# jcorsetti/oryon

Hardware: AMD Instinct MI355X
Metric: image-pairs/sec end-to-end (feat+match+reg) @224², C=256; ADD(-S) parity (higher is better)
Workload: dtype f32

## Files before the change

oryon_amd/csrc/match_corrs.hip:

```cpp
#include <hip/hip_fp16.h>
#include "common.h"
#include "match_common.h"
#include "match_exact.h"

namespace oryon {
constexpr uint8_t LZ_INVALID = 0, LZ_VALID = 1, LZ_UNCERTAIN = 2, LZ_AMB_VALID = 3, LZ_RESOLVED = 4, LZ_AMB_UNCERTAIN = 5;
constexpr uint8_t DC_COMPLETE = 0, DC_SETTLED = 1, DC_OPEN = 2;

struct DcOpenRows {
    const uint8_t *cls = nullptr;
    int S = 0;
    const float *m1 = nullptr;
    const int32_t *i1 = nullptr;
    const float *m2 = nullptr;
    float *r_m1 = nullptr;
    int32_t *r_i1 = nullptr;
    float *r_m2 = nullptr;
};

__device__ __forceinline__ bool decide_lite_row(
    int cap_a, int p, int a, int S, const float *ws_m1, const int32_t *ws_i1,
    const float *ws_m2, const DcOpenRows &open, const float *__restrict__ a_scale8, const float *__restrict__ eps_q8, float cut0, float sqrt_c,
    float c_true, int force_eager, int fmt, int x3, float *__restrict__ m_final, int32_t *__restrict__ sid_final, float *__restrict__ margin_out,
    uint8_t *__restrict__ state, uint8_t *__restrict__ valid, float *__restrict__ min_dist, int32_t *__restrict__ argmin,
// ... 596 lines not shown
    return carve.off;
}

size_t carve_lazy(void *base, LazyWs &w, int B, int C, int cap_a, int cap_q, int S, int corr_rows)
{
    Carver carve(base, carve_screen8_raw(base, w, B, C, cap_a, cap_q, S));
    const size_t rows = (size_t)B * cap_a, pairs = (size_t)B;
    carve(w.margin, rows);
    carve(w.sid_final, rows);
    carve(w.unc_idx, rows);
    carve(w.state, rows);
    carve(w.sel_rows, pairs * corr_rows);
    carve(w.scratch, rows);
    carve(w.n_a_eager, pairs);
    carve(w.n_a_lazy, pairs);
    carve(w.ambu_idx, rows);
    carve(w.ambv_idx, pairs * corr_rows);
    const size_t cap_s = sampled_cap(corr_rows, cap_a);
    const size_t e1 = oryon_match_workspace_bytes(B, cap_a), e2 = oryon_match_workspace_bytes(B, (int)cap_s);
    w.exact_ws_bytes = e1 > e2 ? e1 : e2;
    carve(w.exact_ws, w.exact_ws_bytes > 16 ? w.exact_ws_bytes : 16);
    carve(w.x3_ah, pairs * cap_s * C);
    carve(w.x3_al, pairs * cap_s * C);
    carve(w.x3_a_ovf, pairs * cap_s * C);
    carve(w.x3_md_o, pairs * cap_s);
    carve(w.x3_am_o, pairs * cap_s);
    carve(w.x3_va_o, pairs * cap_s);
    const bool cascade = C == 256 && corr_rows <= MX6_SAMPLED_PANEL;
    const size_t triples = cascade ? pairs * mx6_sampled_splits(B) * MX6_SAMPLED_PANEL : 4;
    carve(w.cs_panel, cascade ? pairs * MX6_SAMPLED_PANEL * C : 16);
    if (!cascade) w.cs_panel = nullptr;
    carve(w.cs_max, triples);
    carve(w.cs_m2, triples);
    carve(w.cs_i1, triples);
    carve(w.n_ambv0, pairs);
    carve(w.cs_gate, pairs * mx6_panels_per_pair(cap_a));
    w.dc_ok = false;
    w.dc_stats = nullptr;
    if (dc_shape(C, cap_a, corr_rows)) {
        LazyWs sized;
        if (carve_dc(nullptr, sized, B, C, cap_a) <= (size_t)B * cap_q * C * sizeof(__half)) {
            carve_dc(w.q16, w, B, C, cap_a);
            w.dc_ok = true;
        }
    }
    w.lazy_zero_off = carve.off;
    carve(w.pair_eager, pairs);
    carve(w.n_unc, pairs);
    carve(w.n_ambu, pairs);
    carve(w.n_ambv, pairs);
    carve(w.need_f32_lazy, pairs);
    carve(w.n_amb_room, pairs);
    w.n_amb_part = w.panel_flag;
    carve(w.mark, rows);
    w.lazy_zero_bytes = carve.off - w.lazy_zero_off;
    w.x3_zero_bytes = match_x3_zero_bytes(B, (int)cap_s, 8);
    carve(w.x3_scratch, match_x3_scratch_bytes(B, (int)cap_s, 8, cap_q));
    return carve.off;
}
}

extern "C" size_t oryon_match_corrs_i8_workspace_bytes(int B, int C, int cap_a, int cap_q, int corr_rows)
{
    if (B <= 0 || C <= 0 || cap_a <= 0 || cap_a % MT16 || cap_q <= 0 || corr_rows <= 0) return 0;
    LazyWs w;
    return carve_lazy(nullptr, w, B, C, cap_a, cap_q, pick_split16(B, cap_a / MT16), corr_rows);
}

int32_t *oryon::match_dc_stats(void *workspace, int B, int C, int cap_a, int cap_q, int corr_rows)
{
    LazyWs w;
    carve_lazy(workspace, w, B, C, cap_a, cap_q, pick_split16(B, cap_a / MT16), corr_rows);
    return w.dc_ok ? w.dc_stats : nullptr;
}

namespace {
constexpr const char *IMPL = "match_corrs_lazy_impl";

SampledAmbList sampled_amb_list(const LazyWs &w)
{
    SampledAmbList L;
    L.state = w.state;
    L.want = LZ_AMB_VALID;
    L.mark = w.mark;
    L.n_list = w.n_ambv;
    L.list = w.ambv_idx;
    return L;
}

int select_step(const MatchCorrsArgs &m, const LazyWs &w, hipStream_t st, const SampledAmbList &amb = SampledAmbList())
{
    const int rc = select_corrs_launch(m.roi_a, m.roi_q, m.roi_stride_a, m.roi_stride_q, m.n_a, m.n_q, m.argmin, m.valid, m.cap_a, m.B, m.W,
                                       m.max_corrs, m.corr_rows, m.seed, m.pair_key, w.scratch, m.corrs, m.n_valid, m.n_sel, m.status,
                                       w.sel_rows, w.pair_eager, st, amb);
    if (rc) set_error("oryon_match_corrs_i8: select launch failed");
    return rc;
}

int eager_route(const MatchCorrsArgs &m, const LazyWs &w, int S)
{
    decide8_step(m, S, w.n_a_eager, w);
    rescore_raw_step(m, w.n_a_eager, 2, w);
    int rc = check_launch(IMPL);
    if (rc) return rc;
    if ((rc = raw_fallbacks(m, w.n_a_eager, w, IMPL, "oryon_match_corrs_i8"))) return rc;
    return select_step(m, w, as_stream(m.stream));
}

void compact_anchors(const MatchCorrsArgs &m, const AnchorRaw &araw, const LazyWs &w, hipStream_t st, int cap_c, const int32_t *count,
                     const int32_t *idx, int idx_stride)
{
    const dim3 grid((cap_c + 63) / 64, m.B);
    if (m.a_hat)
        hipLaunchKernelGGL(match_compact_f32_kernel, grid, dim3(256), 0, st, m.a_hat, m.C, m.cap_a, cap_c, count, idx, idx_stride, w.a_hat_c);
    else
        hipLaunchKernelGGL(m.layout == ORYON_LAYOUT_NHWC ? match_compact_raw_kernel<true> : match_compact_raw_kernel<false>, grid, dim3(256), 0,
                           st, araw, m.C_true, m.HW, m.round_f16, m.C, m.cap_a, cap_c, count, idx, idx_stride, w.a_hat_c);
}

int lazy_route(const MatchCorrsArgs &m, const LazyWs &w, hipStream_t st, int use_x3, bool cascade, bool dc)
{
    const int B = m.B, C = m.C, cap_a = m.cap_a, cap_q = m.cap_q, corr_rows = m.corr_rows;
    const bool nhwc = m.layout == ORYON_LAYOUT_NHWC;
    const AnchorRaw araw = {m.feat_a, m.roi_a, m.a_norm, m.roi_stride_a};
    int rc = gather_q8_launch(m.feat_q, B, m.C_true, m.HW, m.layout, m.roi_q, m.roi_stride_q, m.n_q, w.need_f32_lazy, cap_q, C, w.q8_scratch,
                              w.scale_scratch, w.eps_scratch, nullptr, w.q_hat, 1, m.round_f16, st);
    if (rc) { set_error("oryon_match_corrs_i8: lazy fp32 gather launch failed"); return rc; }
    compact_anchors(m, araw, w, st, cap_a, w.n_ambu, w.ambu_idx, cap_a);
    if ((rc = check_launch(IMPL))) return rc;
    rc = oryon_match_f32(w.a_hat_c, w.q_hat, B, C, cap_a, cap_q, w.n_ambu, m.n_q, m.threshold, w.md_c, w.am_c, w.va_c, w.exact_ws,
                         w.exact_ws_bytes, st);
    if (rc) return rc;
    hipLaunchKernelGGL(match_scatter_exact_kernel, dim3(cap_a / 256, B), dim3(256), 0, st, cap_a, cap_a, w.n_ambu, w.ambu_idx, cap_a, w.md_c,
                       w.am_c, w.va_c, m.min_dist, m.argmin, m.valid, w.state);
    if ((rc = check_launch(IMPL))) return rc;
    const size_t lds_res = (size_t)4 * 2 * C * sizeof(float);
    auto resolve_uncertain = m.fmt == 1 ? (nhwc ? match_resolve_uncertain_kernel<true, 1> : match_resolve_uncertain_kernel<false, 1>)
                                        : (nhwc ? match_resolve_uncertain_kernel<true, 0> : match_resolve_uncertain_kernel<false, 0>);
    hipLaunchKernelGGL(resolve_uncertain, dim3(64, B), dim3(256), lds_res, st, m.a_hat, araw, m.a_i8, m.q_i8, m.q_scale, m.a_scale, m.feat_q,
                       m.C_true, m.HW, m.roi_q, m.roi_stride_q, m.q_norm, C, cap_a, cap_q, m.n_q, m.threshold, w.m_final, w.sid_final, w.margin,
                       w.n_unc, w.unc_idx, w.pair_eager, w.state, m.valid, m.min_dist, m.argmin, m.round_f16);
    if ((rc = check_launch(IMPL))) return rc;
    const SampledAmbList amb = sampled_amb_list(w);
    if ((rc = select_step(m, w, st, amb))) return rc;
    const int cap_s = sampled_cap(corr_rows, cap_a);
    if (cascade) {
        const int csS = mx6_sampled_splits(B);
        launch_screen_mx6_list512(st, reinterpret_cast<const uint8_t *>(m.a_i8), reinterpret_cast<const uint8_t *>(m.q_i8), B, cap_a, MX6_SAMPLED_PANEL,
                                  cap_q, w.n_ambv, w.ambv_idx, corr_rows, 0, m.n_q, csS, w.cs_max, w.cs_i1, w.cs_m2, m.C_true);
        hipLaunchKernelGGL(match_decide_sampled_kernel, dim3(B), dim3(DS_THREADS), 0, st, cap_a, MX6_SAMPLED_PANEL, csS,
                           w.n_ambv, w.ambv_idx, corr_rows, w.cs_max, w.cs_i1, w.cs_m2, m.a_scale, m.q_eps_max, w.m_final, w.sid_final,
                           w.margin, w.state, w.mark, w.n_ambv0, dc ? m.min_dist : nullptr, w.pair_eager, m.n_sel, w.sel_rows, amb);
        if ((rc = check_launch(IMPL))) return rc;
    }
    compact_anchors(m, araw, w, st, cap_s, w.n_ambv, w.ambv_idx, corr_rows);
    if ((rc = check_launch(IMPL))) return rc;
    if (use_x3) {
        __half *qh = reinterpret_cast<__half *>(w.q_hat), *ql = qh + (size_t)B * cap_q * C;
        int32_t *n_ovf = nullptr, *ovf_idx = nullptr;
        rc = match_x3_resolve(w.a_hat_c, w.n_ambv, cap_s, m.feat_q, m.C_true, m.HW, m.layout, m.roi_q, m.roi_stride_q, m.q_norm, m.n_q, B, cap_q,
                              m.threshold, m.round_f16, qh, ql, w.x3_ah, w.x3_al, w.x3_scratch, w.md_c, w.am_c, w.va_c, &n_ovf, &ovf_idx,
                              w.ambv_idx, corr_rows, w.sid_final, cap_a, static_cast<const __half *>(m.q_hi_lo), m.q_lo_sq_max, st);
        if (rc) { set_error("oryon_match_corrs: fp16x3 second-level launch failed"); return rc; }
        rc = gather_q8_launch(m.feat_q, B, m.C_true, m.HW, m.layout, m.roi_q, m.roi_stride_q, m.n_q, n_ovf, cap_q, C, w.q8_scratch,
                              w.scale_scratch, w.eps_scratch, nullptr, w.q_hat, 1, m.round_f16, st);
        if (rc) { set_error("oryon_match_corrs: overflow fp32 gather launch failed"); return rc; }
        hipLaunchKernelGGL(match_compact_f32_kernel, dim3((cap_s + 63) / 64, B), dim3(256), 0, st, w.a_hat_c, C, cap_s, cap_s, n_ovf, ovf_idx,
                           cap_s, w.x3_a_ovf);
        if ((rc = check_launch(IMPL))) return rc;
        rc = oryon_match_f32(w.x3_a_ovf, w.q_hat, B, C, cap_s, cap_q, n_ovf, m.n_q, m.threshold, w.x3_md_o, w.x3_am_o, w.x3_va_o, w.exact_ws,
                             w.exact_ws_bytes, st);
        if (rc) return rc;
        match_x3_scatter_ovf(B, cap_s, n_ovf, ovf_idx, w.x3_md_o, w.x3_am_o, w.x3_va_o, w.md_c, w.am_c, w.va_c, st);
    } else {
        rc = oryon_match_f32(w.a_hat_c, w.q_hat, B, C, cap_s, cap_q, w.n_ambv, m.n_q, m.threshold, w.md_c, w.am_c, w.va_c, w.exact_ws,
                             w.exact_ws_bytes, st);
        if (rc) return rc;
    }
    hipLaunchKernelGGL(match_scatter_exact_kernel, dim3((cap_s + 255) / 256, B), dim3(256), 0, st, cap_a, cap_s, w.n_ambv, w.ambv_idx,
                       corr_rows, w.md_c, w.am_c, w.va_c, m.min_dist, m.argmin, m.valid, w.state);
    if ((rc = check_launch(IMPL))) return rc;
    auto resolve_selected = m.fmt == 1 ? (nhwc ? match_resolve_selected_kernel<true, 1> : match_resolve_selected_kernel<false, 1>)
                                       : (nhwc ? match_resolve_selected_kernel<true, 0> : match_resolve_selected_kernel<false, 0>);
    hipLaunchKernelGGL(resolve_selected, dim3((m.max_corrs + 3) / 4, B), dim3(256), lds_res, st, m.a_hat, araw, m.a_i8, m.q_i8, m.q_scale,
                       m.a_scale, m.feat_q, m.C_true, m.HW, m.roi_q, m.roi_stride_q, m.q_norm, C, cap_a, cap_q, m.n_q, m.W, w.m_final,
                       w.sid_final, w.margin, w.state, w.pair_eager, m.n_sel, w.sel_rows, corr_rows, m.min_dist, m.argmin, m.corrs,
                       m.round_f16);
    if ((rc = check_launch(IMPL))) return rc;
    if (m.n_undecided && cascade) {
        hipLaunchKernelGGL(match_cascade_counts_kernel, dim3((B + 255) / 256), dim3(256), 0, st, B, w.n_amb_part, cap_a / 256, w.n_ambv, w.n_ambv0,
                           m.n_undecided);
        if ((rc = check_launch(IMPL))) return rc;
    } else if (m.n_undecided) {
        hipLaunchKernelGGL(match_sum_counts_kernel, dim3((B + 255) / 256), dim3(256), 0, st, B, w.n_amb, w.n_amb_part, cap_a / 256,
                           m.n_undecided);
        if ((rc = check_launch(IMPL))) return rc;
    }
    return ORYON_OK;
}
}

int oryon::match_corrs_lazy_impl(const MatchCorrsArgs &m)
{
    ORYON_CHECK_ARG((m.a_hat || (m.feat_a && m.a_norm && !m.force_eager)) && m.a_i8 && m.a_scale && m.feat_q && m.roi_a && m.roi_q && m.q_norm && m.q_i8 && m.q_eps_max && m.n_a && m.n_q);
    ORYON_CHECK_ARG((m.fmt == 0 || m.fmt == 1) && (m.fmt == 1 || m.q_scale) && !(m.fmt == 1 && m.force_eager));
    ORYON_CHECK_ARG(!m.q_hi_lo || (m.q_lo_sq_max && m.C == 256));
    ORYON_CHECK_ARG(m.min_dist && m.argmin && m.valid && m.corrs && m.n_valid && m.n_sel && m.status);
    ORYON_CHECK_ARG(m.B >= 0 && (m.C == 256 || m.C == 512) && m.C_true > 0 && m.C_true <= m.C && m.HW > 0 && m.W > 0 && m.max_corrs > 0 && m.corr_rows >= m.max_corrs);
    ORYON_CHECK_ARG(m.layout == ORYON_LAYOUT_NCHW || m.layout == ORYON_LAYOUT_NHWC);
    ORYON_CHECK_ARG(m.cap_a > 0 && m.cap_a % MT16 == 0 && m.cap_q > 0 && m.cap_q % 256 == 0 && m.threshold > 0.0f && m.threshold <= 0.5f);
    if (m.B == 0) return ORYON_OK;
    const int B = m.B, C = m.C, cap_a = m.cap_a, cap_q = m.cap_q;
    const int T = cap_a / MT16;
    const int S = pick_split16(B, T);
    LazyWs w;
    const size_t need = carve_lazy(m.workspace, w, B, C, cap_a, cap_q, S, m.corr_rows);
    if (!m.workspace || m.workspace_bytes < need) {
        set_error("oryon_match_corrs_i8: workspace too small (%zu < %zu)", m.workspace_bytes, need);
        return ORYON_ERR_WORKSPACE;
    }
    hipStream_t st = as_stream(m.stream);
    const float cut0 = 1.0f - 2.0f * m.threshold;
    static const bool x3_env = dev_env_int("ORYON_AMB_X3", 1) != 0;
    const int use_x3 = (x3_env && C == 256 && !m.force_eager) ? 1 : 0;
    ORYON_CHECK_HIP(hipMemsetAsync(static_cast<char *>(m.workspace) + w.zero_off, 0, w.zero_bytes + (w.dc_ok && m.fmt == 1 ? w.dc_zero_bytes : 0), st));
    if (m.force_eager) ORYON_CHECK_HIP(hipMemsetAsync(w.need_f32, 0, (size_t)B * sizeof(int32_t), st));
    ORYON_CHECK_HIP(hipMemsetAsync(static_cast<char *>(m.workspace) + w.lazy_zero_off, 0, w.lazy_zero_bytes + (use_x3 ? w.x3_zero_bytes : 0), st));
    static const bool cascade_env = dev_env_int("ORYON_CASCADE", 1) != 0;
    const bool cascade = cascade_env && m.fmt == 1 && use_x3 && m.q_hi_lo != nullptr && w.cs_panel != nullptr;
    const bool dc = m.cascade != 0 && m.fmt == 1 && use_x3 && m.q_hi_lo == nullptr && w.cs_panel != nullptr && w.dc_ok;
    int S_dec = S;
    const float *dec_m1 = w.ws_max, *dec_m2 = w.ws_m2;
    const int32_t *dec_i1 = w.ws_i1;
    DcOpenRows dc_open;
    if (m.fmt == 1) {
        const uint8_t *a6 = reinterpret_cast<const uint8_t *>(m.a_i8), *q6 = reinterpret_cast<const uint8_t *>(m.q_i8);
        const int groups = ((B * S + 7) / 8) * 8 * T;
        profile_begin(st, screen_mx6_name(C));
        if (cascade) {
            const int T8 = mx6_panels_per_pair(cap_a);
            launch_screen_mx6(C, groups, T, st, a6, q6, B, cap_a, cap_q, m.n_a, m.n_q, S, w.ws_max, w.ws_i1, w.ws_m2, m.C_true, 1, nullptr, 2);
            hipLaunchKernelGGL(match_panel_settle_kernel, dim3(T8, B), dim3(256), 0, st, cap_a, T8, S, m.n_a, w.ws_max, w.ws_m2, m.a_scale,
                               m.q_eps_max, cut0, w.cs_gate);
            launch_screen_mx6(C, groups, T, st, a6, q6, B, cap_a, cap_q, m.n_a, m.n_q, S, w.ws_max, w.ws_i1, w.ws_m2, m.C_true, 1, w.cs_gate, 0);
        } else if (dc) {
            const int T8 = mx6_panels_per_pair(cap_a), stride = dc_probe_stride(cap_a), csS = mx6_sampled_splits(B);
            const int Sb = dc_band_splits(B, cap_a), So = dc_open_splits(B);
            static const int slack = dev_env_int("ORYON_DC_SLACK", DC_SLACK);
            static const int open_panel = dev_env_int("ORYON_DC_OPEN_PANEL", 0) == 1024 ? 1024 : MX6_SAMPLED_PANEL;
            static const int sub_stats = dev_env_int("ORYON_DC_SUB_STATS", 0);
            launch_screen_mx6_list512(st, a6, q6, B, cap_a, MX6_SAMPLED_PANEL, cap_q, m.n_a, nullptr, 0, stride, m.n_q, csS, w.cs_max, w.cs_i1,
                                      w.cs_m2, m.C_true);
            hipLaunchKernelGGL(match_dc_probe_band_kernel, dim3(T8, B), dim3(256), 0, st, cap_a, T8, stride, csS, m.n_a, m.n_q, w.cs_max, w.cs_i1,
                               w.cs_m2, m.a_scale, m.q_eps_max, cut0, w.dc_m1, w.dc_i1, w.dc_m2, w.dc_band, w.dc_stats, slack, sub_stats);
            launch_screen_mx6_band512(st, a6, q6, B, cap_a, cap_q, m.n_a, m.n_q, Sb, w.dc_ws_m1, w.dc_ws_i1, w.dc_ws_m2, m.C_true, w.dc_band, 2 * T8);
            hipLaunchKernelGGL(match_dc_settle_rows_kernel, dim3(B), dim3(DC_SETTLE_THREADS), 0, st, cap_a, T8, stride, Sb, m.n_a, m.n_q, w.dc_ws_m1, w.dc_ws_i1,
                               w.dc_ws_m2, m.a_scale, m.q_eps_max, cut0, w.dc_band, w.dc_m1, w.dc_i1, w.dc_m2, w.dc_cls, w.dc_n_open, w.dc_open_idx,
                               w.dc_stats);
            if (open_panel == 1024) {
                hipLaunchKernelGGL(match_compact_rows_kernel, dim3(cap_a / 16, B), dim3(256), 0, st, a6, C, cap_a, cap_a, w.dc_n_open, w.dc_open_idx,
                                   cap_a, w.dc_rows, open_panel);
                launch_screen_mx6(C, ((B * So + 7) / 8) * 8 * T, T, st, w.dc_rows, q6, B, cap_a, cap_q, w.dc_n_open, m.n_q, So, w.dc_ws_m1, w.dc_ws_i1,
                                  w.dc_ws_m2, m.C_true);
            } else
                launch_screen_mx6_list512(st, a6, q6, B, cap_a, cap_a, cap_q, w.dc_n_open, w.dc_open_idx, cap_a, 0, m.n_q, So, w.dc_ws_m1, w.dc_ws_i1,
                                          w.dc_ws_m2, m.C_true);
            S_dec = 1;
            dec_m1 = w.dc_m1; dec_i1 = w.dc_i1; dec_m2 = w.dc_m2;
            dc_open.cls = w.dc_cls;
            dc_open.S = So;
            dc_open.m1 = w.dc_ws_m1; dc_open.i1 = w.dc_ws_i1; dc_open.m2 = w.dc_ws_m2;
            dc_open.r_m1 = w.dc_m1; dc_open.r_i1 = w.dc_i1; dc_open.r_m2 = w.dc_m2;
        } else {
            launch_screen_mx6(C, groups, T, st, a6, q6, B, cap_a, cap_q, m.n_a, m.n_q, S, w.ws_max, w.ws_i1, w.ws_m2, m.C_true);
        }
        profile_end(st);
    } else {
        screen8_step(m, S, m.n_a, w);
    }
    ORYON_CHECK_LAUNCH();
    hipLaunchKernelGGL(match_decide_lite_kernel, dim3(cap_a / 256, B), dim3(256), 0, st, cap_a, m.n_a, S_dec, dec_m1, dec_i1, dec_m2, dc_open, m.a_scale,
                       m.q_eps_max, cut0, sqrtf((float)m.C_true), (float)m.C_true, m.force_eager, m.fmt, use_x3, w.m_final, w.sid_final, w.margin,
                       w.state, m.valid, m.min_dist, m.argmin, w.pair_eager, w.n_unc, w.unc_idx, w.n_ambu, w.ambu_idx, w.need_f32_lazy,
                       w.n_amb_part);
    if (m.force_eager)
        hipLaunchKernelGGL(match_mask_counts_kernel, dim3((B + 255) / 256), dim3(256), 0, st, B, m.n_a, w.pair_eager, w.n_a_eager, w.n_a_lazy);
    ORYON_CHECK_LAUNCH();
    if (!m.force_eager) return lazy_route(m, w, st, use_x3, cascade || dc, dc);
    const int rc = eager_route(m, w, S);
    if (rc) return rc;
    if (m.n_undecided) ORYON_CHECK_HIP(hipMemcpyAsync(m.n_undecided, w.n_amb, (size_t)B * sizeof(int32_t), hipMemcpyDeviceToDevice, st));
    return ORYON_OK;
}

namespace {
MatchCorrsArgs shared_args(const float *feat_q, int C_true, int HW, int layout, const int32_t *roi_a, int roi_stride_a, const int32_t *roi_q,
                           int roi_stride_q, const float *q_norm, int B, int C, int cap_a, int cap_q, const int32_t *n_a, const int32_t *n_q,
                           float threshold, int W, int max_corrs, int corr_rows, uint64_t seed, const int64_t *pair_key, float *min_dist,
                           int32_t *argmin, uint8_t *valid, int32_t *corrs, int32_t *n_valid, int32_t *n_sel, int32_t *status,
                           int32_t *n_undecided, int round_f16, void *workspace, size_t workspace_bytes, void *stream)
{
    MatchCorrsArgs m;
    m.feat_q = feat_q;
    m.C_true = C_true;
    m.HW = HW;
    m.layout = layout;
// ... 169 lines not shown
```

oryon_amd/csrc/screen_mx6.hip:

```cpp
#include <hip/hip_runtime.h>
#include <stdio.h>
#include <stdlib.h>
#include <type_traits>
#include "common.h"
#include "match_common.h"
#include "screen_tile.h"

namespace oryon {

typedef int i32x8 __attribute__((ext_vector_type(8)));
typedef float f32x16s __attribute__((ext_vector_type(16)));

template <int CP, int WAVES = 8, int VAR = 0>
__global__ __launch_bounds__(64 * WAVES, CP == 512 ? 1 : 2) void match_mx6_screen_kernel(
    const uint8_t *__restrict__ a6, const uint8_t *__restrict__ q6, int B, int cap_a, int cap_q, const int32_t *__restrict__ n_a,
    const int32_t *__restrict__ n_q, int T, int S, float *__restrict__ ws_max, int32_t *__restrict__ ws_i1, float *__restrict__ ws_m2)
{
    constexpr int RB = CP;
    constexpr int TILE_BYTES = screen8_tile_bytes(CP);
    constexpr int NQB = 4, NAB = 2;
    constexpr int NKS = CP / 64;
    constexpr int NI = TILE_BYTES / (1024 * WAVES);
    char *smem;
    if constexpr (2 * TILE_BYTES > 65536) {
        extern __shared__ __attribute__((aligned(256))) char smem_dyn6[];
        smem = smem_dyn6;
    } else {
        __shared__ __attribute__((aligned(256))) char smem_st6[2 * TILE_BYTES];
        smem = smem_st6;
    }
    ScreenUnit u;
    if (!screen_unit_decode(u, 64 * WAVES, B, T, S, n_a, n_q)) return;
    const int p = u.p, split = u.split, a0 = u.a0;
    int qt_begin, qt_end;
    screen_split_tiles(u, S, qt_begin, qt_end);
    const int t = threadIdx.x, lane = t & 63, wave = t >> 6, l31 = lane & 31, hi = lane >> 5;
    const char *qp = reinterpret_cast<const char *>(q6) + (size_t)p * cap_q * RB;

    i32x8 breg[NAB][NKS];
#pragma unroll
    for (int ab = 0; ab < NAB; ++ab) {
        const int arow_i = a0 + wave * 64 + ab * 32 + l31;
        const char *arow = reinterpret_cast<const char *>(a6) + ((size_t)p * cap_a + (arow_i < cap_a ? arow_i : cap_a - 1)) * RB + 32 * hi;
#pragma unroll
        for (int s = 0; s < NKS; ++s) {
            const i32x4 lo = *reinterpret_cast<const i32x4 *>(arow + 64 * s), up = *reinterpret_cast<const i32x4 *>(arow + 64 * s + 16);
            breg[ab][s] = __builtin_shufflevector(lo, up, 0, 1, 2, 3, 4, 5, 6, 7);
        }
    }
    unsigned dma_off[NI];
    screen_dma_offsets<RB>(dma_off, wave * NI, lane);
    const int wave_u = __builtin_amdgcn_readfirstlane(wave);
    auto issue_one = [&](int qt, int buf, int j) {
        const char *qb = qp + (size_t)qt * TILE_BYTES;
        char *dst = smem + buf * TILE_BYTES + (wave_u * NI + j) * 1024;
        __builtin_amdgcn_global_load_lds((const __attribute__((address_space(1))) void *)(qb + dma_off[j]),
                                         (__attribute__((address_space(3))) void *)dst, 16, 0, 0);
    };
    unsigned koff[4][2];
#pragma unroll
    for (int c = 0; c < 4; ++c)
#pragma unroll
        for (int e = 0; e < 2; ++e) koff[c][e] = (unsigned)(l31 * RB) + ((((unsigned)(4 * c + 2 * hi + e)) ^ (unsigned)(l31 & 15)) << 4);
    auto rd = [&](int s, int qb, unsigned tile) -> i32x8 {
        const unsigned base = tile + (unsigned)(qb * 32 * RB + (s >> 2) * 256);
        const i32x4 lo = *reinterpret_cast<const i32x4 *>(smem + koff[s & 3][0] + base);
        const i32x4 up = *reinterpret_cast<const i32x4 *>(smem + koff[s & 3][1] + base);
        return __builtin_shufflevector(lo, up, 0, 1, 2, 3, 4, 5, 6, 7);
    };

    float runmax[NAB], run2[NAB];
    int runidx[NAB];
#pragma unroll
    for (int ab = 0; ab < NAB; ++ab) { runmax[ab] = -INFINITY; run2[ab] = -INFINITY; runidx[ab] = 0; }
    auto reduce_block = [&](const f32x16s &c, int sid, int ab) {
        if constexpr (VAR == 1) { runmax[ab] = fmaxf(runmax[ab], c[0] + c[15]); runidx[ab] = sid; return; }
        const float m0 = fmaxf(fmaxf(c[0], c[1]), c[2]), m1 = fmaxf(fmaxf(c[3], c[4]), c[5]), m2 = fmaxf(fmaxf(c[6], c[7]), c[8]);
        const float m3 = fmaxf(fmaxf(c[9], c[10]), c[11]), m4 = fmaxf(fmaxf(c[12], c[13]), c[14]);
        const float x = fmaxf(fmaxf(fmaxf(m0, m1), m2), fmaxf(fmaxf(m3, m4), c[15]));
        const bool improved = x > runmax[ab];
        run2[ab] = __builtin_amdgcn_fmed3f(runmax[ab], run2[ab], x);
        runmax[ab] = fmaxf(runmax[ab], x);
        runidx[ab] = improved ? sid : runidx[ab];
    };
    const f32x16s zero16 = {0, 0, 0, 0, 0, 0, 0, 0, 0, 0, 0, 0, 0, 0, 0, 0};

    if (qt_end > qt_begin) {
#pragma unroll
        for (int j = 0; j < NI; ++j) issue_one(qt_begin, 0, j);
    }
    asm volatile("s_waitcnt vmcnt(0)" ::: "memory");
    __syncthreads();

    i32x8 areg[NKS];
#pragma unroll
    for (int s = 0; s < NKS; ++s) areg[s] = rd(s, 0, 0u);
    f32x16s prev[NAB];
#pragma unroll
    for (int ab = 0; ab < NAB; ++ab)
#pragma unroll
        for (int r = 0; r < 16; ++r) prev[ab][r] = -3.0e38f;
    int prev_sid = 0;
    auto do_tile = [&](int qt, auto BUFC) {
        constexpr int BUF = decltype(BUFC)::value;
        constexpr unsigned tile = BUF * TILE_BYTES;
        const int qt_next = qt + 1 < qt_end ? qt + 1 : qt;
#pragma unroll
        for (int qb = 0; qb < NQB; ++qb) {
            f32x16s acc[NAB];
            if (qb == 0) {
#pragma unroll
                for (int j = 0; j < NI; ++j) issue_one(qt_next, BUF ^ 1, j);
            }
#pragma unroll
            for (int s = 0; s < NKS; ++s) {
#pragma unroll
                for (int ab = 0; ab < NAB; ++ab)
                    acc[ab] = __builtin_amdgcn_mfma_scale_f32_32x32x64_f8f6f4(areg[s], breg[ab][s], s == 0 ? zero16 : acc[ab], 2, 2, 0,
                                                                               areg[s][6], 0, breg[ab][s][6]);
                if (qb + 1 < NQB) areg[s] = rd(s, qb + 1, tile);
            }
#pragma unroll
            for (int ab = 0; ab < NAB; ++ab) reduce_block(prev[ab], prev_sid, ab);
#pragma unroll
            for (int i = 0; i < NKS; ++i) {
                __builtin_amdgcn_sched_group_barrier(0x008, 1, 0);
                __builtin_amdgcn_sched_group_barrier(0x002, 24 / (2 * NKS), 0);
                __builtin_amdgcn_sched_group_barrier(0x008, 1, 0);
                __builtin_amdgcn_sched_group_barrier(0x002, 24 / (2 * NKS), 0);
                if (qb + 1 < NQB) __builtin_amdgcn_sched_group_barrier(0x100, 2, 0);
            }
#pragma unroll
            for (int ab = 0; ab < NAB; ++ab) prev[ab] = acc[ab];
            prev_sid = (qt * NQB + qb) * 2 + hi;
        }
        asm volatile("s_waitcnt vmcnt(0)" ::: "memory");
        __syncthreads();
#pragma unroll
        for (int s = 0; s < NKS; ++s) areg[s] = rd(s, 0, (BUF ^ 1) * TILE_BYTES);
    };
    for (int qt = qt_begin; qt < qt_end; qt += 2) {
        do_tile(qt, std::integral_constant<int, 0>{});
        if (qt + 1 < qt_end) do_tile(qt + 1, std::integral_constant<int, 1>{});
    }
#pragma unroll
    for (int ab = 0; ab < NAB; ++ab) reduce_block(prev[ab], prev_sid, ab);
    screen_merge_store<NAB>(runmax, run2, runidx, a0 + wave * 64 + l31, hi, (size_t)p * S + split, cap_a, ws_max, ws_i1, ws_m2);
}


template <int S0, int N, class F>
__device__ __forceinline__ void mx6_static_for(F &&f)
{
    if constexpr (S0 < N) {
        f(std::integral_constant<int, S0>{});
        mx6_static_for<S0 + 1, N>(f);
    }
}

struct Mx6RowList {
    const int32_t *idx;
    int idx_stride, stride, cap_src;
    int n;
};
struct Mx6RowsInPlace {};

template <int CP, int WAVES, int KL, bool IDX = false>
__device__ __forceinline__ void mx6_screen_w4_tiles(char *smem, const uint8_t *__restrict__ a6, const uint8_t *__restrict__ q6, int p, int split,
                                                    int a0, int cap_a, int cap_q, int S, int qt_begin, int qt_end, float *__restrict__ ws_max,
                                                    int32_t *__restrict__ ws_i1, float *__restrict__ ws_m2,
                                                    const std::conditional_t<IDX, Mx6RowList, Mx6RowsInPlace> &rows = {})
{
    static_assert(CP == 256 || (CP == 512 && WAVES == 4), "geometries: C_pad 256 with 4 / 8 waves, C_pad 512 with 4 waves");
    constexpr int RB = CP, NAB = 4;
    constexpr int TILE_BYTES = screen8_tile_bytes(CP);
    constexpr int NQB = 4;
    constexpr int NKS = CP / 64;
    constexpr int NI = TILE_BYTES / (1024 * WAVES);
    constexpr int LPR = RB / 256;
    const int t = threadIdx.x, lane = t & 63, wave = t >> 6, l31 = lane & 31, hi = lane >> 5;
    const char *qp = reinterpret_cast<const char *>(q6) + (size_t)p * cap_q * RB;

    i32x8 breg[NAB][NKS];
    int bsc[NAB][NKS / 4];
#pragma unroll
    for (int ab = 0; ab < NAB; ++ab) {
        const int arow_i = a0 + wave * (32 * NAB) + ab * 32 + l31;
        const char *arow;
        bool live = true;
        if constexpr (IDX) {
            live = arow_i < rows.n;
            const int src = !live ? 0 : rows.idx ? rows.idx[(size_t)p * rows.idx_stride + arow_i] : arow_i * rows.stride;
            arow = reinterpret_cast<const char *>(a6) + ((size_t)p * rows.cap_src + src) * RB + 32 * hi;
        } else
            arow = reinterpret_cast<const char *>(a6) + ((size_t)p * cap_a + (arow_i < cap_a ? arow_i : cap_a - 1)) * RB + 32 * hi;
        unsigned sc[NKS / 4];
#pragma unroll
        for (int w = 0; w < NKS / 4; ++w) sc[w] = 0;
#pragma unroll
        for (int s = 0; s < KL; ++s) {
            i32x4 lo = *reinterpret_cast<const i32x4 *>(arow + 64 * s), up = *reinterpret_cast<const i32x4 *>(arow + 64 * s + 16);
            if constexpr (IDX) {
                const i32x4 z = {0, 0, 0, 0};
                lo = live ? lo : z;
                up = live ? up : z;
            }
            breg[ab][s] = __builtin_shufflevector(lo, up, 0, 1, 2, 3, 4, 5, -1, -1);
            sc[s >> 2] |= ((unsigned)up[2] & 0xffu) << (8 * (s & 3));
        }
#pragma unroll
        for (int w = 0; w < NKS / 4; ++w) bsc[ab][w] = (int)sc[w];
    }
    constexpr int DJ = 4 * LPR;
    static_assert(NI % DJ == 0 || NI == DJ, "DMA instructions per wave and tile");
    unsigned dma_off[DJ];
    screen_dma_offsets<RB>(dma_off, wave * NI, lane);
    const int wave_u = __builtin_amdgcn_readfirstlane(wave);
    auto issue_one = [&](int qt, int buf, int j) {
        const char *qb = qp + (size_t)qt * TILE_BYTES + (j / DJ) * (16 * RB);
        char *dst = smem + buf * TILE_BYTES + (wave_u * NI + j) * 1024;
        __builtin_amdgcn_global_load_lds((const __attribute__((address_space(1))) void *)(qb + dma_off[j % DJ]),
                                         (__attribute__((address_space(3))) void *)dst, 16, 0, 0);
    };
    unsigned koff[4][2];
#pragma unroll
    for (int c = 0; c < 4; ++c)
#pragma unroll
        for (int e = 0; e < 2; ++e) koff[c][e] = (unsigned)(l31 * RB) + ((((unsigned)(4 * c + 2 * hi + e)) ^ (unsigned)(l31 & 15)) << 4);
    auto rd = [&](int s, int qb, unsigned tile) -> i32x8 {
        const unsigned base = tile + (unsigned)(qb * 32 * RB + (s >> 2) * 256);
        const i32x4 lo = *reinterpret_cast<const i32x4 *>(smem + koff[s & 3][0] + base);
        const i32x4 up = *reinterpret_cast<const i32x4 *>(smem + koff[s & 3][1] + base);
        return __builtin_shufflevector(lo, up, 0, 1, 2, 3, 4, 5, 6, -1);
    };

    float runmax[NAB], run2[NAB];
    int runidx[NAB];
#pragma unroll
    for (int ab = 0; ab < NAB; ++ab) { runmax[ab] = -INFINITY; run2[ab] = -INFINITY; runidx[ab] = 0; }
    auto reduce_block = [&](const f32x16s &c, int sid, int ab) {
        const float m0 = fmaxf(fmaxf(c[0], c[1]), c[2]), m1 = fmaxf(fmaxf(c[3], c[4]), c[5]), m2 = fmaxf(fmaxf(c[6], c[7]), c[8]);
        const float m3 = fmaxf(fmaxf(c[9], c[10]), c[11]), m4 = fmaxf(fmaxf(c[12], c[13]), c[14]);
        const float x = fmaxf(fmaxf(fmaxf(m0, m1), m2), fmaxf(fmaxf(m3, m4), c[15]));
        const bool improved = x > runmax[ab];
        run2[ab] = __builtin_amdgcn_fmed3f(runmax[ab], run2[ab], x);
        runmax[ab] = __builtin_amdgcn_fmed3f(runmax[ab], x, INFINITY);
        runidx[ab] = improved ? sid : runidx[ab];
    };
    const f32x16s zero16 = {0, 0, 0, 0, 0, 0, 0, 0, 0, 0, 0, 0, 0, 0, 0, 0};

    if (qt_end > qt_begin) {
#pragma unroll
        for (int j = 0; j < NI; ++j) issue_one(qt_begin, 0, j);
    }
    asm volatile("s_waitcnt vmcnt(0)" ::: "memory");
    __syncthreads();

    i32x8 areg[NKS];
#pragma unroll
    for (int s = 0; s < KL; ++s) areg[s] = rd(s, 0, 0u);
    f32x16s acc[NAB];
#pragma unroll
    for (int ab = 0; ab < NAB; ++ab)
#pragma unroll
        for (int r = 0; r < 16; ++r) acc[ab][r] = -3.0e38f;
    int sid23 = 0;

    auto mfma = [&](f32x16s &d, int ab, auto SC) {
        constexpr int s_ = decltype(SC)::value;
        d = __builtin_amdgcn_mfma_scale_f32_32x32x64_f8f6f4(areg[s_], breg[ab][s_], s_ == 0 ? zero16 : d, 2, 2, 0, areg[s_][6], s_ & 3,
                                                            bsc[ab][s_ >> 2]);
    };
    int buf = 0;
    for (int qt = qt_begin; qt < qt_end; ++qt) {
        const unsigned tile = buf * TILE_BYTES;
        const int qt_next = qt + 1 < qt_end ? qt + 1 : qt;
#pragma unroll
        for (int qb = 0; qb < NQB; ++qb) {
            const int sid = (qt * NQB + qb) * 2 + hi;
            if (qb == 0) {
#pragma unroll
                for (int j = 0; j < NI; ++j) issue_one(qt_next, buf ^ 1, j);
            }
            reduce_block(acc[2], sid23, 2);
            reduce_block(acc[3], sid23, 3);
            mx6_static_for<0, KL>([&](auto SC) { mfma(acc[0], 0, SC); mfma(acc[1], 1, SC); });
#pragma unroll
            for (int i = 0; i < 2 * KL; ++i) {
                __builtin_amdgcn_sched_group_barrier(0x008, 1, 0);
                __builtin_amdgcn_sched_group_barrier(0x002, 16 / KL, 0);
            }
            mx6_static_for<0, KL>([&](auto SC) {
                constexpr int s_ = decltype(SC)::value;
                mfma(acc[2], 2, SC); mfma(acc[3], 3, SC);
                if (qb + 1 < NQB) areg[s_] = rd(s_, qb + 1, tile);
            });
            reduce_block(acc[0], sid, 0);
            reduce_block(acc[1], sid, 1);
#pragma unroll
            for (int i = 0; i < 2 * KL; ++i) {
                __builtin_amdgcn_sched_group_barrier(0x008, 1, 0);
                __builtin_amdgcn_sched_group_barrier(0x002, 16 / KL, 0);
                if (qb + 1 < NQB && (i & 1)) __builtin_amdgcn_sched_group_barrier(0x100, 2, 0);
            }
            sid23 = sid;
        }
        asm volatile("s_waitcnt vmcnt(0)" ::: "memory");
        __syncthreads();
        buf ^= 1;
#pragma unroll
        for (int s = 0; s < KL; ++s) areg[s] = rd(s, 0, buf * TILE_BYTES);
    }
    reduce_block(acc[2], sid23, 2);
    reduce_block(acc[3], sid23, 3);
    screen_merge_store<NAB>(runmax, run2, runidx, a0 + wave * (32 * NAB) + l31, hi, (size_t)p * S + split, cap_a, ws_max, ws_i1, ws_m2);
}

template <int CP, int WAVES, int KL = CP / 64>
__global__ __launch_bounds__(64 * WAVES, CP == 512 ? 1 : 2) void match_mx6_screen_w4_kernel(
    const uint8_t *__restrict__ a6, const uint8_t *__restrict__ q6, int B, int cap_a, int cap_q, const int32_t *__restrict__ n_a,
    const int32_t *__restrict__ n_q, int T, int S, float *__restrict__ ws_max, int32_t *__restrict__ ws_i1, float *__restrict__ ws_m2,
    long long *__restrict__ dbg_wg )
{
    constexpr int TILE_BYTES = screen8_tile_bytes(CP);
    char *smem;
    if constexpr (2 * TILE_BYTES > 65536) {
        extern __shared__ __attribute__((aligned(256))) char smem_dyn_w4[];
        smem = smem_dyn_w4;
    } else {
        __shared__ __attribute__((aligned(256))) char smem_st_w4[2 * TILE_BYTES];
        smem = smem_st_w4;
    }
    ScreenUnit u;
    if (!screen_unit_decode(u, 128 * WAVES, B, T, S, n_a, n_q)) return;
    int qt_begin, qt_end;
    screen_split_tiles(u, S, qt_begin, qt_end);
    const long long tk0 = dbg_wg ? wall_clock64() : 0;
    mx6_screen_w4_tiles<CP, WAVES, KL>(smem, a6, q6, u.p, u.split, u.a0, cap_a, cap_q, S, qt_begin, qt_end, ws_max, ws_i1, ws_m2);
    if (dbg_wg && threadIdx.x == 0) {
        dbg_wg[(size_t)blockIdx.x * 4 + 0] = tk0;
        dbg_wg[(size_t)blockIdx.x * 4 + 1] = wall_clock64();
        dbg_wg[(size_t)blockIdx.x * 4 + 2] = (long long)__builtin_amdgcn_s_getreg((31 << 11) | 4);
        dbg_wg[(size_t)blockIdx.x * 4 + 3] = (long long)__builtin_amdgcn_s_getreg((31 << 11) | 20);
    }
}

template <int KL>
__global__ __launch_bounds__(256, 2) void match_mx6_screen_w4_list_kernel(
    const uint8_t *__restrict__ a6, const uint8_t *__restrict__ q6, int B, int cap_src, int cap_list, int cap_q, const int32_t *__restrict__ count,
    const int32_t *__restrict__ idx, int idx_stride, int stride, const int32_t *__restrict__ n_q, int T, int S, float *__restrict__ ws_max,
    int32_t *__restrict__ ws_i1, float *__restrict__ ws_m2)
{
    __shared__ __attribute__((aligned(256))) char smem_st_w4l[2 * screen8_tile_bytes(256)];
    ScreenUnit u;
    if (!screen_unit_decode(u, 512, B, T, S, count, n_q)) return;
    Mx6RowList rows = {idx, idx_stride, stride, cap_src, 0};
    const int listed = idx ? u.na : (u.na + stride - 1) / stride;
    rows.n = listed < cap_list ? listed : cap_list;
    if (u.a0 >= rows.n) return;
    int qt_begin, qt_end;
    screen_split_tiles(u, S, qt_begin, qt_end);
    mx6_screen_w4_tiles<256, 4, KL, true>(smem_st_w4l, a6, q6, u.p, u.split, u.a0, cap_list, cap_q, S, qt_begin, qt_end, ws_max, ws_i1, ws_m2, rows);
}

template <int CP, int WAVES, int KL = CP / 64>
__global__ __launch_bounds__(64 * WAVES, CP == 512 ? 1 : 2) void match_mx6_screen_w4_win_kernel(
    const uint8_t *__restrict__ a6, const uint8_t *__restrict__ q6, int B, int cap_a, int cap_q, const int32_t *__restrict__ n_a,
    const int32_t *__restrict__ n_q, int T, int S, float *__restrict__ ws_max, int32_t *__restrict__ ws_i1, float *__restrict__ ws_m2,
    const int32_t *__restrict__ gate , int win ,
    const int32_t *__restrict__ band ,
    int band_T )
{
    constexpr int TILE_BYTES = screen8_tile_bytes(CP);
    char *smem;
    if constexpr (2 * TILE_BYTES > 65536) {
        extern __shared__ __attribute__((aligned(256))) char smem_dyn_w4w[];
        smem = smem_dyn_w4w;
    } else {
        __shared__ __attribute__((aligned(256))) char smem_st_w4w[2 * TILE_BYTES];
        smem = smem_st_w4w;
    }
    ScreenUnit u;
    if (!screen_unit_decode(u, 128 * WAVES, B, T, S, n_a, n_q)) return;
    if (gate && gate[u.p * T + u.panel] == 0) return;
    int qt_begin, qt_end;
    screen_split_tiles(u, S, qt_begin, qt_end);
    if (win > 0 && qt_end - qt_begin > win) {
        const int cnt = qt_end - qt_begin, panels = (u.na + 128 * WAVES - 1) / (128 * WAVES);
        int k0 = (int)(((long long)(2 * u.panel + 1) * cnt) / (2 * panels)) - win / 2;
        k0 = k0 < 0 ? 0 : (k0 > cnt - win ? cnt - win : k0);
        qt_begin += k0;
        qt_end = qt_begin + win;
    }
    if (band) {
        const int first = band[(u.p * band_T + u.panel) * 2], cnt = band[(u.p * band_T + u.panel) * 2 + 1];
        const int per = (cnt + S - 1) / S;
        qt_begin = first + u.split * per;
        qt_end = (qt_begin + per < first + cnt) ? qt_begin + per : first + cnt;
    }
    mx6_screen_w4_tiles<CP, WAVES, KL>(smem, a6, q6, u.p, u.split, u.a0, cap_a, cap_q, S, qt_begin, qt_end, ws_max, ws_i1, ws_m2);
}

static void mx6_debug_report(const long long *dbg_dev, int groups, hipStream_t st)
{
    (void)hipStreamSynchronize(st);
    long long *w = static_cast<long long *>(malloc((size_t)groups * 4 * sizeof(long long)));
    (void)hipMemcpy(w, dbg_dev, (size_t)groups * 4 * sizeof(long long), hipMemcpyDeviceToHost);
    long long t0 = -1, t1 = 0;
    double sum = 0;
    int ran = 0;
    long long longest = 0;
    for (int g = 0; g < groups; ++g)
        if (w[4 * g + 1]) {
            if (t0 < 0 || w[4 * g] < t0) t0 = w[4 * g];
            if (w[4 * g + 1] > t1) t1 = w[4 * g + 1];
            sum += (double)(w[4 * g + 1] - w[4 * g]);
            if (w[4 * g + 1] - w[4 * g] > longest) longest = w[4 * g + 1] - w[4 * g];
            ++ran;
        }
    fprintf(stderr, "[mx6] %d of %d workgroups ran: span %.1f us, mean %.1f us, longest %.1f us, mean residency %.1f workgroups\n", ran, groups,
            (t1 - t0) * 0.01, ran ? sum * 0.01 / ran : 0.0, longest * 0.01, t1 > t0 ? sum / (double)(t1 - t0) : 0.0);
    fprintf(stderr, "[mx6] resident at 5%%..95%% of the span:");
    for (int k = 0; k < 10; ++k) {
        const long long ts = t0 + (t1 - t0) * (2 * k + 1) / 20;
        int r = 0;
        for (int g = 0; g < groups; ++g) r += w[4 * g + 1] && w[4 * g] <= ts && ts < w[4 * g + 1];
        fprintf(stderr, " %d", r);
    }
    fprintf(stderr, "\n");
    free(w);
}

static int mx6_var()
{
    static const int var = dev_env_int("ORYON_MX6_VAR", 0);
    return var;
}

namespace {
int mx6_live_ksteps(int C_true) { return (C_true > 0 && C_true <= 64) ? 1 : (C_true > 0 && C_true <= 128) ? 2 : 4; }
template <class F>
void mx6_with_kl(int kl, F &&f)
{
    if (kl == 1) f(std::integral_constant<int, 1>{});
    else if (kl == 2) f(std::integral_constant<int, 2>{});
    else f(std::integral_constant<int, 4>{});
}

template <int CP>
void launch_screen_mx6_t(int groups, int T, hipStream_t st, const uint8_t *a6, const uint8_t *q6, int B, int cap_a, int cap_q, const int32_t *n_a,
                       const int32_t *n_q, int S, float *ws_max, int32_t *ws_i1, float *ws_m2, int kl = 4, bool gate_or_win = false,
                       const int32_t *gate = nullptr, int win = 0)
{
    constexpr size_t dyn = 2 * screen8_tile_bytes(CP) > 65536 ? 2 * screen8_tile_bytes(CP) : 0;
    constexpr int W_ = CP == 512 ? 4 : 8;
    const int Tw = (cap_a + 64 * W_ - 1) / (64 * W_);
    const int var = mx6_var();
    if (var == 1) {
        if (dyn) allow_dynamic_lds(reinterpret_cast<const void *>(&match_mx6_screen_kernel<CP, W_, 1>), (int)dyn);
        hipLaunchKernelGGL((match_mx6_screen_kernel<CP, W_, 1>), dim3(groups / T * Tw), dim3(64 * W_), dyn, st, a6, q6, B, cap_a, cap_q, n_a, n_q, Tw,
                           S, ws_max, ws_i1, ws_m2);
        return;
    }
    if constexpr (CP == 256) {
        if (var == 0) {
            const int T8 = (cap_a + 1023) / 1024;
            static const bool dbg = dev_env_set("ORYON_MX6_DEBUG");
            static long long *dbg_wg = nullptr;
            const int g8 = groups / T * T8;
            if (dbg && !dbg_wg) (void)hipMalloc(&dbg_wg, (size_t)65536 * 4 * sizeof(long long));
            if (dbg && dbg_wg && g8 <= 65536) (void)hipMemsetAsync(dbg_wg, 0, (size_t)g8 * 4 * sizeof(long long), st);
            if (gate_or_win) {
                mx6_with_kl(kl, [&](auto KLC) {
                    hipLaunchKernelGGL((match_mx6_screen_w4_win_kernel<CP, 8, decltype(KLC)::value>), dim3(g8), dim3(512), 0, st, a6, q6, B, cap_a,
                                       cap_q, n_a, n_q, T8, S, ws_max, ws_i1, ws_m2, gate, win, static_cast<const int32_t *>(nullptr), 0);
                });
                return;
            }
            mx6_with_kl(kl, [&](auto KLC) {
                hipLaunchKernelGGL((match_mx6_screen_w4_kernel<CP, 8, decltype(KLC)::value>), dim3(g8), dim3(512), 0, st, a6, q6, B, cap_a, cap_q,
                                   n_a, n_q, T8, S, ws_max, ws_i1, ws_m2, (dbg && g8 <= 65536) ? dbg_wg : nullptr);
            });
            if (dbg && dbg_wg && g8 <= 65536) mx6_debug_report(dbg_wg, g8, st);
            return;
        }
        if (var == 3) {
            hipLaunchKernelGGL((match_mx6_screen_w4_kernel<CP, 4>), dim3(groups / T * Tw), dim3(256), 0, st, a6, q6, B, cap_a, cap_q, n_a, n_q, Tw, S,
                               ws_max, ws_i1, ws_m2, nullptr);
            return;
        }
    }
    if constexpr (CP == 512) {
        if (var == 0) {
            allow_dynamic_lds(reinterpret_cast<const void *>(&match_mx6_screen_w4_kernel<CP, 4>), (int)dyn);
            hipLaunchKernelGGL((match_mx6_screen_w4_kernel<CP, 4>), dim3(groups / T * Tw), dim3(256), dyn, st, a6, q6, B, cap_a, cap_q, n_a, n_q, Tw,
                               S, ws_max, ws_i1, ws_m2, nullptr);
            return;
        }
    }
    if (dyn) allow_dynamic_lds(reinterpret_cast<const void *>(&match_mx6_screen_kernel<CP, W_>), (int)dyn);
    hipLaunchKernelGGL((match_mx6_screen_kernel<CP, W_>), dim3(groups / T * Tw), dim3(64 * W_), dyn, st, a6, q6, B, cap_a, cap_q, n_a, n_q, Tw, S,
                       ws_max, ws_i1, ws_m2);
}
}

const char *screen_mx6_name(int C)
{
    if (C != 256) return mx6_var() == 0 ? "match_mx6_screen_w4_kernel<512, 4>" : "match_mx6_screen_kernel<512, 4, 0>";
    return mx6_var() == 0 ? "match_mx6_screen_w4_kernel<256, 8>" : mx6_var() == 3 ? "match_mx6_screen_w4_kernel<256, 4>" : mx6_var() == 1 ? "match_mx6_screen_kernel<256, 8, 1>" : "match_mx6_screen_kernel<256, 8, 0>";
}

void launch_screen_mx6(int C, int groups, int T, hipStream_t st, const uint8_t *a6, const uint8_t *q6, int B, int cap_a, int cap_q,
                       const int32_t *n_a, const int32_t *n_q, int S, float *ws_max, int32_t *ws_i1, float *ws_m2, int C_true,
                       int cascade, const int32_t *gate, int win)
{
// ... 31 lines not shown
```

oryon_amd/csrc/screen_tile.h:

```cpp
#pragma once
#include <hip/hip_runtime.h>
#include <stdint.h>

namespace oryon {

typedef int i32x4 __attribute__((ext_vector_type(4)));

constexpr int SCREEN8_ROWS = 128;
constexpr int screen8_tile_bytes(int CP) { return CP * SCREEN8_ROWS; }

struct ScreenUnit {
    int p, split, panel, a0, na, nq;
};
__device__ __forceinline__ bool screen_unit_decode(ScreenUnit &u, int panel_rows, int B, int T, int S, const int32_t *__restrict__ n_a,
                                                   const int32_t *__restrict__ n_q)
{
    const int xcd = blockIdx.x & 7, slot = blockIdx.x >> 3;
    const int unit = (slot / T) * 8 + xcd;
    if (unit >= B * S) return false;
    u.panel = slot % T;
    u.p = unit / S;
    u.split = unit % S;
    u.na = n_a[u.p];
    u.nq = n_q[u.p];
    u.a0 = u.panel * panel_rows;
    return u.a0 < u.na;
}
__device__ __forceinline__ void screen_split_tiles(const ScreenUnit &u, int S, int &qt_begin, int &qt_end)
{
    const int nqt = (u.nq + SCREEN8_ROWS - 1) / SCREEN8_ROWS;
    const int qt_per = (nqt + S - 1) / S;
    qt_begin = u.split * qt_per;
    qt_end = (qt_begin + qt_per < nqt) ? qt_begin + qt_per : nqt;
}

template <int RB, int N>
__device__ __forceinline__ void screen_dma_offsets(unsigned (&off)[N], int first, int lane)
{
    constexpr int LPR = RB / 256;
    static_assert(LPR >= 1, "rows are whole 256-byte lines");
#pragma unroll
    for (int j = 0; j < N; ++j) {
        const int line = (first + j) * 4 + (lane >> 4), sl = lane & 15;
        const int row = line / LPR;
        off[j] = (unsigned)(row * RB + (((line % LPR) * 16 + (sl ^ (row & 15))) << 4));
    }
}

template <int NAB>
__device__ __forceinline__ void screen_merge_store(const float (&runmax)[NAB], const float (&run2)[NAB], const int (&runidx)[NAB], int a_lane,
                                                   int hi, size_t unit, int cap_a, float *__restrict__ ws_max, int32_t *__restrict__ ws_i1,
                                                   float *__restrict__ ws_m2)
{
#pragma unroll
    for (int ab = 0; ab < NAB; ++ab) {
        const float om1 = __shfl_xor(runmax[ab], 32), om2 = __shfl_xor(run2[ab], 32);
        const int oi1 = __shfl_xor(runidx[ab], 32);
        const float m1 = fmaxf(runmax[ab], om1);
        const float m2 = fmaxf(fminf(runmax[ab], om1), fmaxf(run2[ab], om2));
        const int i1 = (om1 > runmax[ab]) ? oi1 : runidx[ab];
        const int a = a_lane + ab * 32;
        if (hi == 0 && a < cap_a) {
            const size_t o = unit * cap_a + a;
            ws_max[o] = m1;
            ws_i1[o] = i1;
            ws_m2[o] = m2;
        }
    }
}

}
```

Measured before the change: 24010.

## Specialize list-panel MX6 screen on live row blocks to skip empty MFMA work

The list-indexed MX6 screen kernel now interleaves panel rows across waves (block stride 128) and picks a template instantiation with 1-4 row blocks per wave based on how many list rows are live in the panel. Partially filled panels then skip MFMAs and reductions on empty row blocks, and the sched_group_barrier interleaving is generalised to uneven halves. The change also adds an env-gated debug print of sampled-list sizes, which syncs the stream when enabled. It adds template instances and code size, and the new row mapping must stay consistent with the store stride.

```diff
diff --git a/oryon_amd/csrc/match_corrs.hip b/oryon_amd/csrc/match_corrs.hip
--- a/oryon_amd/csrc/match_corrs.hip
+++ b/oryon_amd/csrc/match_corrs.hip
@@ -772,6 +772,17 @@
                            w.n_ambv, w.ambv_idx, corr_rows, w.cs_max, w.cs_i1, w.cs_m2, m.a_scale, m.q_eps_max, w.m_final, w.sid_final,
                            w.margin, w.state, w.mark, w.n_ambv0, dc ? m.min_dist : nullptr, w.pair_eager, m.n_sel, w.sel_rows, amb);
         if ((rc = check_launch(IMPL))) return rc;
+        static const bool print_lists = dev_env_set("ORYON_PRINT_SAMPLED_LIST");
+        if (print_lists) {
+            int32_t *h = static_cast<int32_t *>(malloc((size_t)B * sizeof(int32_t)));
+            (void)hipStreamSynchronize(st);
+            (void)hipMemcpy(h, w.n_ambv0, (size_t)B * sizeof(int32_t), hipMemcpyDeviceToHost);
+            long long sum = 0;
+            int lo = h[0], hi = h[0], le384 = 0;
+            for (int p = 0; p < B; ++p) { sum += h[p]; lo = h[p] < lo ? h[p] : lo; hi = h[p] > hi ? h[p] : hi; le384 += h[p] <= 384; }
+            fprintf(stderr, "[sampled list] rows per pair: mean %.1f, min %d, max %d; %d of %d pairs at most 384 rows\n", (double)sum / B, lo, hi, le384, B);
+            free(h);
+        }
     }
     compact_anchors(m, araw, w, st, cap_s, w.n_ambv, w.ambv_idx, corr_rows);
     if ((rc = check_launch(IMPL))) return rc;
diff --git a/oryon_amd/csrc/screen_mx6.hip b/oryon_amd/csrc/screen_mx6.hip
--- a/oryon_amd/csrc/screen_mx6.hip
+++ b/oryon_amd/csrc/screen_mx6.hip
@@ -165,14 +165,16 @@
 };
 struct Mx6RowsInPlace {};
 
-template <int CP, int WAVES, int KL, bool IDX = false>
+template <int CP, int WAVES, int KL, bool IDX = false, int NBL = 4>
 __device__ __forceinline__ void mx6_screen_w4_tiles(char *smem, const uint8_t *__restrict__ a6, const uint8_t *__restrict__ q6, int p, int split,
                                                     int a0, int cap_a, int cap_q, int S, int qt_begin, int qt_end, float *__restrict__ ws_max,
                                                     int32_t *__restrict__ ws_i1, float *__restrict__ ws_m2,
                                                     const std::conditional_t<IDX, Mx6RowList, Mx6RowsInPlace> &rows = {})
 {
     static_assert(CP == 256 || (CP == 512 && WAVES == 4), "geometries: C_pad 256 with 4 / 8 waves, C_pad 512 with 4 waves");
-    constexpr int RB = CP, NAB = 4;
+    static_assert(NBL == 4 || (IDX && NBL >= 1 && NBL < 4), "fewer live blocks: list panels only");
+    constexpr int RB = CP, NAB = NBL;
+    constexpr int NH0 = (NAB + 1) / 2, NH1 = NAB - NH0;
     constexpr int TILE_BYTES = screen8_tile_bytes(CP);
     constexpr int NQB = 4;
     constexpr int NKS = CP / 64;
@@ -185,7 +187,7 @@
     int bsc[NAB][NKS / 4];
 #pragma unroll
     for (int ab = 0; ab < NAB; ++ab) {
-        const int arow_i = a0 + wave * (32 * NAB) + ab * 32 + l31;
+        const int arow_i = a0 + (IDX ? list_panel_row(wave, ab, l31) : wave * (32 * NAB) + ab * 32 + l31);
         const char *arow;
         bool live = true;
         if constexpr (IDX) {
@@ -271,6 +273,10 @@
         d = __builtin_amdgcn_mfma_scale_f32_32x32x64_f8f6f4(areg[s_], breg[ab][s_], s_ == 0 ? zero16 : d, 2, 2, 0, areg[s_][6], s_ & 3,
                                                             bsc[ab][s_ >> 2]);
     };
+    auto reduce_h1 = [&](int sid_) {
+        if constexpr (NH1 > 0) reduce_block(acc[NH0], sid_, NH0);
+        if constexpr (NH1 > 1) reduce_block(acc[NH0 + 1], sid_, NH0 + 1);
+    };
     int buf = 0;
     for (int qt = qt_begin; qt < qt_end; ++qt) {
         const unsigned tile = buf * TILE_BYTES;
@@ -282,26 +288,33 @@
 #pragma unroll
                 for (int j = 0; j < NI; ++j) issue_one(qt_next, buf ^ 1, j);
             }
-            reduce_block(acc[2], sid23, 2);
-            reduce_block(acc[3], sid23, 3);
-            mx6_static_for<0, KL>([&](auto SC) { mfma(acc[0], 0, SC); mfma(acc[1], 1, SC); });
-#pragma unroll
-            for (int i = 0; i < 2 * KL; ++i) {
-                __builtin_amdgcn_sched_group_barrier(0x008, 1, 0);
-                __builtin_amdgcn_sched_group_barrier(0x002, 16 / KL, 0);
+            reduce_h1(sid23);
+            mx6_static_for<0, KL>([&](auto SC) {
+                mfma(acc[0], 0, SC);
+                if constexpr (NH0 > 1) mfma(acc[1], 1, SC);
+            });
+            if constexpr (NH1 > 0) {
+#pragma unroll
+                for (int i = 0; i < NH0 * KL; ++i) {
+                    __builtin_amdgcn_sched_group_barrier(0x008, 1, 0);
+                    __builtin_amdgcn_sched_group_barrier(0x002, 16 * NH1 / (NH0 * KL), 0);
+                }
             }
             mx6_static_for<0, KL>([&](auto SC) {
                 constexpr int s_ = decltype(SC)::value;
-                mfma(acc[2], 2, SC); mfma(acc[3], 3, SC);
+                if constexpr (NH1 > 0) mfma(acc[NH0], NH0, SC);
+                if constexpr (NH1 > 1) mfma(acc[NH0 + 1], NH0 + 1, SC);
                 if (qb + 1 < NQB) areg[s_] = rd(s_, qb + 1, tile);
             });
             reduce_block(acc[0], sid, 0);
-            reduce_block(acc[1], sid, 1);
-#pragma unroll
-            for (int i = 0; i < 2 * KL; ++i) {
-                __builtin_amdgcn_sched_group_barrier(0x008, 1, 0);
-                __builtin_amdgcn_sched_group_barrier(0x002, 16 / KL, 0);
-                if (qb + 1 < NQB && (i & 1)) __builtin_amdgcn_sched_group_barrier(0x100, 2, 0);
+            if constexpr (NH0 > 1) reduce_block(acc[1], sid, 1);
+            if constexpr (NH1 > 0) {
+#pragma unroll
+                for (int i = 0; i < NH1 * KL; ++i) {
+                    __builtin_amdgcn_sched_group_barrier(0x008, 1, 0);
+                    __builtin_amdgcn_sched_group_barrier(0x002, 16 * NH0 / (NH1 * KL), 0);
+                    if (qb + 1 < NQB && (i + 1) % NH1 == 0) __builtin_amdgcn_sched_group_barrier(0x100, 2, 0);
+                }
             }
             sid23 = sid;
         }
@@ -311,9 +324,12 @@
 #pragma unroll
         for (int s = 0; s < KL; ++s) areg[s] = rd(s, 0, buf * TILE_BYTES);
     }
-    reduce_block(acc[2], sid23, 2);
-    reduce_block(acc[3], sid23, 3);
-    screen_merge_store<NAB>(runmax, run2, runidx, a0 + wave * (32 * NAB) + l31, hi, (size_t)p * S + split, cap_a, ws_max, ws_i1, ws_m2);
+    reduce_h1(sid23);
+    if constexpr (IDX)
+        screen_merge_store<NAB>(runmax, run2, runidx, a0 + list_panel_row(wave, 0, l31), hi, (size_t)p * S + split, cap_a, ws_max, ws_i1, ws_m2,
+                                LIST_BLOCK_STRIDE);
+    else
+        screen_merge_store<NAB>(runmax, run2, runidx, a0 + wave * (32 * NAB) + l31, hi, (size_t)p * S + split, cap_a, ws_max, ws_i1, ws_m2);
 }
 
 template <int CP, int WAVES, int KL = CP / 64>
@@ -360,7 +376,15 @@
     if (u.a0 >= rows.n) return;
     int qt_begin, qt_end;
     screen_split_tiles(u, S, qt_begin, qt_end);
-    mx6_screen_w4_tiles<256, 4, KL, true>(smem_st_w4l, a6, q6, u.p, u.split, u.a0, cap_list, cap_q, S, qt_begin, qt_end, ws_max, ws_i1, ws_m2, rows);
+    auto run = [&](auto NBLC) {
+        mx6_screen_w4_tiles<256, 4, KL, true, decltype(NBLC)::value>(smem_st_w4l, a6, q6, u.p, u.split, u.a0, cap_list, cap_q, S, qt_begin, qt_end,
+                                                                      ws_max, ws_i1, ws_m2, rows);
+    };
+    const int nbl = list_panel_nbl(rows.n - u.a0);
+    if (nbl >= 4) run(std::integral_constant<int, 4>{});
+    else if (nbl == 3) run(std::integral_constant<int, 3>{});
+    else if (nbl == 2) run(std::integral_constant<int, 2>{});
+    else run(std::integral_constant<int, 1>{});
 }
 
 template <int CP, int WAVES, int KL = CP / 64>
diff --git a/oryon_amd/csrc/screen_tile.h b/oryon_amd/csrc/screen_tile.h
--- a/oryon_amd/csrc/screen_tile.h
+++ b/oryon_amd/csrc/screen_tile.h
@@ -47,10 +47,21 @@
     }
 }
 
+constexpr int LIST_PANEL_ROWS = 512;
+struct ListRowPlace {
+    int wave, slot, lane;
+};
+constexpr ListRowPlace list_row_place(int r) { return {(r >> 5) & 3, r >> 7, r & 31}; }
+constexpr int list_panel_row(int wave, int slot, int lane) { return slot * 128 + wave * 32 + lane; }
+constexpr int list_live_blocks(int m) { return ((m < LIST_PANEL_ROWS ? m : LIST_PANEL_ROWS) + 31) >> 5; }
+constexpr int list_wave_blocks(int m, int wave) { return (list_live_blocks(m) + 3 - wave) >> 2; }
+constexpr int list_panel_nbl(int m) { return (list_live_blocks(m) + 3) >> 2; }
+constexpr int LIST_BLOCK_STRIDE = 128;
+
 template <int NAB>
 __device__ __forceinline__ void screen_merge_store(const float (&runmax)[NAB], const float (&run2)[NAB], const int (&runidx)[NAB], int a_lane,
                                                    int hi, size_t unit, int cap_a, float *__restrict__ ws_max, int32_t *__restrict__ ws_i1,
-                                                   float *__restrict__ ws_m2)
+                                                   float *__restrict__ ws_m2, int block_stride = 32)
 {
 #pragma unroll
     for (int ab = 0; ab < NAB; ++ab) {
@@ -59,7 +70,7 @@
         const float m1 = fmaxf(runmax[ab], om1);
         const float m2 = fmaxf(fminf(runmax[ab], om1), fmaxf(run2[ab], om2));
         const int i1 = (om1 > runmax[ab]) ? oi1 : runidx[ab];
-        const int a = a_lane + ab * 32;
+        const int a = a_lane + ab * block_stride;
         if (hi == 0 && a < cap_a) {
             const size_t o = unit * cap_a + a;
             ws_max[o] = m1;
```

Result: no change. 24190 (median of 6 runs) (+0.8%).
